# snap-research/GiGL

Measured on AMD Instinct MI355X. Metric: sampled+aggregated edges/s, higher is better.
Workload: dtype f32

## Files before the change

### gigl_amd/csrc/sample.hip

```cpp
#include "common.h"

#include <cstdlib>
#include <mutex>
#include <type_traits>

namespace {

constexpr uint64_t P1 = 0x9E3779B185EBCA87ULL;
constexpr uint64_t P2 = 0xC2B2AE3D27D4EB4FULL;
constexpr uint64_t P3 = 0x165667B19E3779F9ULL;
constexpr uint64_t P5 = 0x27D4EB2F165667C5ULL;
constexpr uint64_t SPARK_SEED = 42ULL;
constexpr uint64_t SIGN = 0x8000000000000000ULL;

__device__ __forceinline__ uint64_t xxh64_i32_ordered(uint32_t x) {
  uint64_t h = (SPARK_SEED + P5 + 4ULL) ^ ((uint64_t)x * P1);
  h = ((h << 23) | (h >> 41)) * P2 + P3;
  h ^= h >> 33;
  h *= P2;
  h ^= h >> 29;
  h *= P3;
  h ^= h >> 32;
  return h ^ SIGN;
}
// ... 225 lines not shown
    } else {
      const uint32_t ulo = dpp_shr1((uint32_t)key), uhi = dpp_shr1((uint32_t)(key >> 32));
      const uint32_t ui = dpp_shr1(idx), gtu = dpp_shr1(gt ? 1u : 0u);
      if (gtu) {
        key = ((uint64_t)uhi << 32) | ulo;
        idx = ui;
      } else if (gt) {
        key = ck;
        idx = ci;
      }
    }
  }
  __device__ __forceinline__ void merge(key_t ck, uint32_t ci, bool valid) {
    if constexpr (FAST) {
      if (__ballot(valid && ck == tk && tk != inf())) tie = true;
    }
    unsigned long long m = __ballot(valid && lt(ck, ci, tk, ti));
    while (m) {
      const int src = __ffsll((long long)m) - 1;
      m &= m - 1;
      const key_t sk = bcast(ck, src);
      const uint32_t si = readlane32(ci, src);
      if constexpr (FAST) {
        if (sk == tk) tie = true;
      }
      if (lt(sk, si, tk, ti)) {
        insert(sk, si);
        refresh_threshold();
      }
    }
  }
  __device__ __forceinline__ void scan_row(const uint32_t* flat, int64_t deg, uint32_t base) {
    const int64_t nchunks = (deg + 63) >> 6;
    const uint32_t* src = flat + base;
    auto key_at = [&](int64_t i) -> key_t {
      if constexpr (FAST) {
        if (flat) return i <= deg ? (key_t)(src[i] & dmask) : inf();
      }
      return mk(xxh64_i32_ordered((uint32_t)i + base));
    };
    int64_t c = 0;
    for (; c + 3 < nchunks; c += 4) {
      const int64_t ia = 1 + c * 64 + lane, ib = ia + 64, ic = ib + 64, id = ic + 64;
      const key_t ka = key_at(ia), kb = key_at(ib), kc = key_at(ic), kd = key_at(id);
      merge(ka, (uint32_t)ia, ia <= deg);
      merge(kb, (uint32_t)ib, ib <= deg);
      merge(kc, (uint32_t)ic, ic <= deg);
      merge(kd, (uint32_t)id, id <= deg);
    }
    for (; c < nchunks; ++c) {
      const int64_t i = 1 + c * 64 + lane;
      merge(key_at(i), (uint32_t)i, i <= deg);
    }
  }
  __device__ __forceinline__ bool scan_level(const RangeTable& tb, int l, uint32_t T, uint32_t n, uint32_t base) {
    const int gs = TBL_IDX_SHIFT + l;
    const uint32_t* off = tb.off[l];
    const uint2* ent = tb.lvl[l];
    const uint32_t start = off[(base + 1u) >> gs], end = off[((base + n) >> gs) + 1u];
    for (uint32_t e0 = start; e0 < end; e0 += 64u) {
      const uint32_t e = e0 + (uint32_t)lane;
      uint2 x = make_uint2(0u, 0xFFFFFFFFu);
      if (e < end) x = ent[e];
      const uint32_t i = x.x - base;
      const bool pass = e < end && (uint32_t)(i - 1u) < n && x.y < T;
      key_t ck;
      if constexpr (FAST) ck = x.y & dmask;
      else ck = xxh64_i32_ordered(x.x);
      merge(ck, i, pass);
    }
    return readlane32(idx, f - 1) != 0xFFFFFFFFu;
  }
  __device__ __forceinline__ bool finish(uint32_t count, uint32_t* lk, uint32_t* li) {
    if (count < (uint32_t)f || count > 64u) {
      wave_lds_sync();
      return false;
    }
    if (lane < 7) lk[count + (uint32_t)lane] = 0xFFFFFFFFu;
    wave_lds_sync();
    const bool valid = (uint32_t)lane < count;
    const uint32_t k = valid ? lk[lane] : 0xFFFFFFFFu;
    const uint32_t i = valid ? li[lane] : 0xFFFFFFFFu;
    uint32_t rank = 0;
    for (uint32_t j = 0; j < count; j += 8) {
      const uint4 q = *(const uint4*)(lk + j), r = *(const uint4*)(lk + j + 4);
      rank += (q.x < k ? 1u : 0u) + (q.y < k ? 1u : 0u) + (q.z < k ? 1u : 0u) + (q.w < k ? 1u : 0u);
      rank += (r.x < k ? 1u : 0u) + (r.y < k ? 1u : 0u) + (r.z < k ? 1u : 0u) + (r.w < k ? 1u : 0u);
    }
    wave_lds_sync();
    selmask = __ballot(valid && rank < (uint32_t)f);
    if (__popcll(selmask) != f) {
      tie = true;
      return true;
    }
    idx = i;
    ordered = true;
    return true;
  }
  __device__ __forceinline__ void offer(uint32_t k, uint32_t i, bool pass, uint32_t& count, uint32_t* lk, uint32_t* li) {
    const unsigned long long m = __ballot(pass);
    const uint32_t pos =
        count + __builtin_amdgcn_mbcnt_hi((uint32_t)(m >> 32), __builtin_amdgcn_mbcnt_lo((uint32_t)m, 0u));
    if (pass && pos < 64u) {
      lk[pos] = k;
      li[pos] = i;
    }
    count += (uint32_t)__popcll(m);
  }
  template <int SRC>
  __device__ __forceinline__ bool filter_positions(const uint32_t* flat, uint32_t n, uint32_t T, uint32_t base,
                                                   uint32_t* lk, uint32_t* li) {
    const bool all = T == 0xFFFFFFFFu;
    uint32_t count = 0;
    const uint32_t nchunks = (n + 63u) >> 6;
    const uint32_t* src = flat + base;
    for (uint32_t c = 0; c < nchunks; c += 4) {
      uint32_t kk[4];
#pragma unroll
      for (uint32_t t = 0; t < 4; ++t) {
        const uint32_t i = (c + t) * 64u + (uint32_t)lane + 1u;
        kk[t] = 0xFFFFFFFFu;
        if constexpr (SRC == SRC_FLAT) {
          if (c + t < nchunks) kk[t] = src[i];
        } else {
          kk[t] = (uint32_t)(xxh64_i32_ordered(i + base) >> 32);
        }
      }
#pragma unroll
      for (uint32_t t = 0; t < 4; ++t) {
        if (c + t >= nchunks) break;
        const uint32_t i = (c + t) * 64u + (uint32_t)lane + 1u;
        const uint32_t k = kk[t] & dmask;
        offer(k, i, i <= n && (all || k < T), count, lk, li);
      }
    }
    return finish(count, lk, li);
  }
  __device__ __forceinline__ bool filter_level(const uint2* ent, uint32_t cnt, uint32_t n, uint32_t T, uint32_t base,
                                               uint32_t* lk, uint32_t* li) {
    uint32_t count = 0;
    for (uint32_t e0 = 0; e0 < cnt; e0 += 128u) {
      const uint32_t ea = e0 + (uint32_t)lane, eb = ea + 64u;
      uint2 xa = make_uint2(0u, 0xFFFFFFFFu), xb = xa;
      if (ea < cnt) xa = ent[ea];
      if (eb < cnt) xb = ent[eb];
      const uint32_t ia = xa.x - base, ib = xb.x - base;
      offer(xa.y & dmask, ia, (uint32_t)(ia - 1u) < n && xa.y < T, count, lk, li);
      if (e0 + 64u < cnt) offer(xb.y & dmask, ib, (uint32_t)(ib - 1u) < n && xb.y < T, count, lk, li);
    }
    return finish(count, lk, li);
  }
  __device__ __forceinline__ void serial(const RangeTable& tb, uint32_t n, uint32_t base, uint32_t T, bool in_table) {
    reset_best();
    if (!in_table) {
      scan_row(nullptr, (int64_t)n, base);
      return;
    }
    const uint32_t T4 = T >= (1u << 30) ? 0xFFFFFFFFu : 4u * T;
    const int l4 = T4 == 0xFFFFFFFFu ? 0 : min((int)__builtin_clz(T4 - 1u), tb.levels);
    if (l4 > 0) {
      if (scan_level(tb, l4, T4, n, base)) return;
      reset_best();
    }
    if constexpr (FAST) {
      scan_row(tb.flat, (int64_t)n, base);
      if (readlane32(idx, f - 1) == 0xFFFFFFFFu) tie = true;
    } else {
      scan_row(nullptr, (int64_t)n, base);
    }
  }
};

enum { ROW_INVALID = 0, ROW_COPY = 1, ROW_FLAT = 2, ROW_LEVEL = 3, ROW_HASH = 4, ROW_SERIAL = 5, ROW_SERIAL_HASH = 6,
       ROW_SKIP = 7 };

struct __attribute__((aligned(32))) RowDesc {
  int64_t s;
  uint32_t n;
  uint32_t base;
  uint32_t T;
  uint32_t kind_cnt;
  const void* ptr;
};

__device__ __forceinline__ float filter_lambda(int f) { return (float)f + 4.f * __builtin_sqrtf((float)f) + 4.f; }

constexpr int WORK_LISTS = 64;
constexpr int WORK_CNT_STRIDE = 32;

struct WorkLists {
  uint32_t* items;
  int32_t* count;
  int64_t cap;
  int32_t iters;
  int32_t wgs;
};

__host__ __device__ static inline int64_t work_list_cap(int64_t n_parents) {
  return ((n_parents / 256 + 1 + WORK_LISTS - 1) / WORK_LISTS) * 256;
}
static inline int64_t expand_desc_bytes(int64_t n_parents) {
  return (n_parents + 1) * (int64_t)sizeof(RowDesc) + WORK_LISTS * work_list_cap(n_parents) * 4 +
         WORK_LISTS * WORK_CNT_STRIDE * 4 + 512;
}

__global__ void work_counts_zero_kernel(int32_t* count) { count[threadIdx.x * WORK_CNT_STRIDE] = 0; }

__global__ __launch_bounds__(256) void plan_rows_kernel(ExpandArgs a, RangeTable tb, RowDesc* __restrict__ desc,
                                                        int64_t* heavy_list, int32_t* heavy_count, WorkLists wl) {
  __shared__ int32_t s_wave[4];
  __shared__ int32_t s_base;
  const uint32_t p = blockIdx.x * 256u + threadIdx.x;
  const int lane = threadIdx.x & 63, w = threadIdx.x >> 6;
  bool real = false;
  if (p <= (uint32_t)a.n_parents) {
    RowDesc d{};
    if (p == (uint32_t)a.n_parents) {
      d.kind_cnt = ROW_SKIP;
      desc[p] = d;
    } else {
      uint32_t v, ksum;
      parent_of(a, p, v, ksum);
      uint32_t* out = a.out_nbr + (int64_t)p * a.f;
      if (v == GIGL_INVALID || (int64_t)v >= a.n_nodes) {
        for (int j = 0; j < a.f; ++j) out[j] = GIGL_INVALID;
        a.out_cnt[p] = 0;
      } else {
        int64_t deg;
        if (a.peer_world) {
          const uint32_t q = v / a.peer_world, rk = v - q * a.peer_world;
          const int64_t* rp = a.peer_rowptr[rk];
          const int64_t s0 = rp[q];
          deg = rp[q + 1] - s0;
          d.s = ((int64_t)rk << 48) | s0;
        } else {
          d.s = a.rowptr[v];
          deg = a.rowptr[v + 1] - d.s;
        }
        d.n = (uint32_t)deg;
        d.base = ksum + (uint32_t)a.hash_add;
        if (deg <= a.f && !a.multi) {
          const uint32_t* row = row_of_desc(a, d.s);
          for (int j = 0; j < a.f; ++j) out[j] = j < (int)deg ? row[j] : GIGL_INVALID;
          a.out_cnt[p] = (int32_t)deg;
        } else if (deg <= a.f) {
          d.kind_cnt = ROW_COPY;
          desc[p] = d;
          real = true;
        } else {
          const bool in_table = (uint64_t)d.base + (uint64_t)deg < tb.dom;
          const float lam = filter_lambda(a.f);
          d.T = d.n <= 64u ? 0xFFFFFFFFu
                           : (uint32_t)fminf(lam * 4294967296.f * __builtin_amdgcn_rcpf((float)d.n), 4294967040.f);
          uint32_t kind;
          if (!in_table) {
            if (deg > HEAVY_DEG) {
              kind = ROW_SKIP;
              if (heavy_list) heavy_list[atomicAdd(heavy_count, 1)] = (int64_t)p;
            } else {
              kind = lam <= 56.f ? ROW_HASH : ROW_SERIAL_HASH;
            }
          } else if (lam > 56.f) {
            kind = ROW_SERIAL;
          } else {
            const int l = min((int)__builtin_clz(d.T - 1u), tb.levels);
            if (l == 0 || d.n <= (uint32_t)a.flat_max) {
              kind = ROW_FLAT;
              d.ptr = tb.flat;
            } else {
              const int gs = TBL_IDX_SHIFT + l;
              const uint32_t* off = tb.off[l];
              const uint32_t start = off[(d.base + 1u) >> gs], end = off[((d.base + d.n) >> gs) + 1u];
              if (end - start > 256u) {
                kind = ROW_SERIAL;
              } else {
                kind = ROW_LEVEL | ((end - start) << 3);
                d.ptr = tb.lvl[l] + start;
              }
            }
          }
          d.kind_cnt = kind;
          desc[p] = d;
          real = (kind & 7u) != ROW_SKIP;
        }
      }
    }
  }
  const unsigned long long m = __ballot(real);
  if (lane == 0) s_wave[w] = (int32_t)__popcll(m);
  __syncthreads();
  const int list = (int)(blockIdx.x % WORK_LISTS);
  if (threadIdx.x == 0) {
    const int32_t tot = s_wave[0] + s_wave[1] + s_wave[2] + s_wave[3];
    s_base = tot ? atomicAdd(&wl.count[list * WORK_CNT_STRIDE], tot) : 0;
  }
  __syncthreads();
  if (real) {
    int32_t pos = s_base + (int32_t)__popcll(m & ((1ull << lane) - 1ull));
    for (int k = 0; k < w; ++k) pos += s_wave[k];
    wl.items[(int64_t)list * wl.cap + pos] = p;
  }
}

struct Cand {
  uint32_t k0, j0, k1, j1;
  bool ahead;
};

__device__ __forceinline__ Cand fetch_candidates(const RowDesc& d, int lane) {
  Cand c;
  c.k0 = c.k1 = 0xFFFFFFFFu;
  c.j0 = c.j1 = d.base;
  c.ahead = false;
  const uint32_t kind = d.kind_cnt & 7u, cnt = d.kind_cnt >> 3;
  if (kind == ROW_LEVEL && cnt <= 128u) {
    const uint2* ent = (const uint2*)d.ptr;
    if ((uint32_t)lane < cnt) {
      const uint2 x = ent[lane];
      c.j0 = x.x;
      c.k0 = x.y;
    }
    if ((uint32_t)lane + 64u < cnt) {
      const uint2 x = ent[lane + 64];
      c.j1 = x.x;
      c.k1 = x.y;
    }
    c.ahead = true;
  } else if (kind == ROW_FLAT && d.n <= 128u) {
    const uint32_t* src = (const uint32_t*)d.ptr + d.base;
    c.j0 = d.base + (uint32_t)lane + 1u;
    c.k0 = src[lane + 1];
    if (d.n > 64u) {
      c.j1 = c.j0 + 64u;
      c.k1 = src[lane + 65];
    }
    c.ahead = true;
  }
  return c;
}

__device__ __forceinline__ bool select_ahead(Sel<true>& sel, const RowDesc& d, const Cand& c, uint32_t* lk, uint32_t* li) {
  const uint32_t n = d.n, T = d.T, base = d.base;
  const bool all = T == 0xFFFFFFFFu;
  uint32_t count = 0;
  const uint32_t i0 = c.j0 - base, i1 = c.j1 - base;
  sel.offer(c.k0 & sel.dmask, i0, (uint32_t)(i0 - 1u) < n && (all || c.k0 < T), count, lk, li);
  if ((d.kind_cnt & 7u) == ROW_LEVEL ? (d.kind_cnt >> 3) > 64u : n > 64u)
    sel.offer(c.k1 & sel.dmask, i1, (uint32_t)(i1 - 1u) < n && (all || c.k1 < T), count, lk, li);
  return sel.finish(count, lk, li);
}

__global__ __launch_bounds__(256) __attribute__((amdgpu_waves_per_eu(8, 8))) void expand_rows_kernel(
    ExpandArgs a, RangeTable tb, const RowDesc* __restrict__ desc, WorkLists wl) {
  __shared__ __attribute__((aligned(16))) uint32_t s_lk[4][72], s_li[4][64];
  const int lane = threadIdx.x & 63;
  const int wave_in_block = __builtin_amdgcn_readfirstlane((int)(threadIdx.x >> 6));
  const int f = a.f;
  uint32_t* lk = s_lk[wave_in_block];
  uint32_t* li = s_li[wave_in_block];
  const uint32_t wgs_p = wl.iters > 0 ? (uint32_t)wl.wgs : gridDim.x;
  const uint32_t round = blockIdx.x / wgs_p;
  const uint32_t gw = (blockIdx.x % wgs_p) * 4u + (uint32_t)wave_in_block, n_waves = wgs_p * 4u;
  const uint32_t list = gw % WORK_LISTS, stride = n_waves / WORK_LISTS;
  const int32_t n_items = __builtin_amdgcn_readfirstlane(wl.count[list * WORK_CNT_STRIDE]);
  const uint32_t* items = wl.items + (int64_t)list * wl.cap;
  const uint32_t k_first = gw / WORK_LISTS + stride * round * (uint32_t)wl.iters;
  const uint32_t k_end = wl.iters > 0 ? k_first + stride * (uint32_t)wl.iters : 0xFFFFFFFFu;
  for (uint32_t k = k_first; (int32_t)(2u * k) < n_items && k < k_end; k += stride) {
    const uint32_t p0 = __builtin_amdgcn_readfirstlane(items[2u * k]);
    const uint32_t p1 = (int32_t)(2u * k + 1u) < n_items ? __builtin_amdgcn_readfirstlane(items[2u * k + 1u])
                                                         : (uint32_t)a.n_parents;
    const RowDesc d0 = desc[p0], d1 = desc[p1];
    const Cand c0 = fetch_candidates(d0, lane), c1 = fetch_candidates(d1, lane);
    Sel<true> s0, s1;
    s0.init(f, lane, a.proxy_drop);
    s1.init(f, lane, a.proxy_drop);
    const bool done0 = c0.ahead && !a.multi && select_ahead(s0, d0, c0, lk, li) && !s0.tie;
    uint32_t slot0 = 0, val0 = 0;
    bool sel0 = false;
    if (done0) {
      const unsigned long long m = s0.selmask;
      sel0 = (m >> lane) & 1ull;
      slot0 = __builtin_amdgcn_mbcnt_hi((uint32_t)(m >> 32), __builtin_amdgcn_mbcnt_lo((uint32_t)m, 0u));
      if (sel0) val0 = row_of_desc(a, d0.s)[s0.idx - 1];
    }
    const bool done1 = c1.ahead && !a.multi && select_ahead(s1, d1, c1, lk, li) && !s1.tie;
    uint32_t slot1 = 0, val1 = 0;
    bool sel1 = false;
    if (done1) {
      const unsigned long long m = s1.selmask;
      sel1 = (m >> lane) & 1ull;
      slot1 = __builtin_amdgcn_mbcnt_hi((uint32_t)(m >> 32), __builtin_amdgcn_mbcnt_lo((uint32_t)m, 0u));
      if (sel1) val1 = row_of_desc(a, d1.s)[s1.idx - 1];
    }
    if (done0) {
      if (sel0) a.out_nbr[(int64_t)p0 * f + slot0] = val0;
      if (lane == 0) a.out_cnt[p0] = f;
    }
    if (done1) {
      if (sel1) a.out_nbr[(int64_t)p1 * f + slot1] = val1;
      if (lane == 0) a.out_cnt[p1] = f;
    }
    if (done0 && done1) continue;
  #pragma nounroll
    for (int r = 0; r < 2; ++r) {
      if (r == 0 ? done0 : done1) continue;
      const RowDesc d = r == 0 ? d0 : d1;
      const uint32_t p = r == 0 ? p0 : p1;
      const uint32_t kind = d.kind_cnt & 7u;
      if (kind == ROW_SKIP) continue;
      uint32_t* out = a.out_nbr + (int64_t)p * f;
      if (kind == ROW_INVALID) {
        if (lane < f) out[lane] = GIGL_INVALID;
        if (lane == 0) a.out_cnt[p] = 0;
        continue;
      }
      const uint32_t* row = row_of_desc(a, d.s);
      const uint32_t n = d.n, base = d.base, T = d.T;
      if (kind == ROW_COPY) {
        if (a.multi) {
          const int nw = emit_sorted_distinct(row, (uint32_t)lane < n ? (uint32_t)lane + 1u : 0xFFFFFFFFu, f, lane, out);
          if (lane == 0) a.out_cnt[p] = nw;
          continue;
        }
        if (lane < f) out[lane] = (uint32_t)lane < n ? row[lane] : GIGL_INVALID;
        if (lane == 0) a.out_cnt[p] = (int32_t)n;
        continue;
      }
      const bool in_table = kind != ROW_HASH && kind != ROW_SERIAL_HASH;
      uint32_t sel_idx;
      {
        Sel<true> fast;
        fast.init(f, lane, a.proxy_drop);
        bool done = false;
        if (kind == ROW_LEVEL) done = fast.filter_level((const uint2*)d.ptr, d.kind_cnt >> 3, n, T, base, lk, li);
        else if (kind == ROW_FLAT) done = fast.template filter_positions<SRC_FLAT>((const uint32_t*)d.ptr, n, T, base, lk, li);
        else if (kind == ROW_HASH) done = fast.template filter_positions<SRC_HASH>(nullptr, n, T, base, lk, li);
        if (!done) fast.serial(tb, n, base, T, in_table);
        sel_idx = fast.idx;
        if (fast.tie) {
          Sel<false> exact;
          exact.init(f, lane);
          exact.serial(tb, n, base, T, in_table);
          sel_idx = exact.idx;
        } else if (fast.ordered) {
          const unsigned long long m = fast.selmask;
          const bool sel = (m >> lane) & 1ull;
          const uint32_t slot = __builtin_amdgcn_mbcnt_hi((uint32_t)(m >> 32), __builtin_amdgcn_mbcnt_lo((uint32_t)m, 0u));
          const uint32_t val = sel ? row[sel_idx - 1] : GIGL_INVALID;
          if (!a.multi) {
            if (sel) out[slot] = val;
            if (lane == 0) a.out_cnt[p] = f;
            continue;
          }
          if (sel) lk[slot] = val;
          wave_lds_sync();
          const bool keep = sel && (slot == 0 || lk[slot - 1] != val);
          wave_lds_sync();
          const unsigned long long km = __ballot(keep);
          if (lane < f) out[lane] = GIGL_INVALID;
          if (keep) out[__builtin_amdgcn_mbcnt_hi((uint32_t)(km >> 32), __builtin_amdgcn_mbcnt_lo((uint32_t)km, 0u))] = val;
          if (lane == 0) a.out_cnt[p] = (int32_t)__popcll(km);
          continue;
        }
      }
      if (a.multi) {
        const int nw = emit_sorted_distinct(row, sel_idx, f, lane, out);
        if (lane == 0) a.out_cnt[p] = nw;
        continue;
      }
      emit_sorted(row, sel_idx, f, lane, out);
      if (lane == 0) a.out_cnt[p] = f;
    }
    wave_lds_sync();
  }
}

__global__ __launch_bounds__(256) void table_flat_kernel(uint32_t* flat, uint64_t dom) {
  const uint64_t j = (uint64_t)blockIdx.x * 256 + threadIdx.x;
  if (j < dom) flat[j] = (uint32_t)(xxh64_i32_ordered((uint32_t)j) >> 32);
}

__device__ __forceinline__ int level_of(uint32_t proxy, int levels) { return min((int)__clz((int)proxy), levels); }

__global__ __launch_bounds__(256) void table_count_kernel(const uint32_t* flat, uint32_t* cnt, uint32_t n_tiles,
                                                          int levels) {
  __shared__ uint32_t s_cnt[TBL_MAX_LEVELS + 1][4];
  const int lane = threadIdx.x & 63, w = threadIdx.x >> 6;
  const uint32_t tile = blockIdx.x;
  const uint64_t j0 = ((uint64_t)tile << TBL_TILE_SHIFT) + (uint64_t)w * 256 + lane;
  int m[4];
#pragma unroll
  for (int r = 0; r < 4; ++r) m[r] = level_of(flat[j0 + r * 64], levels);
  for (int l = 1; l <= levels; ++l) {
    uint32_t c = 0;
#pragma unroll
    for (int r = 0; r < 4; ++r) c += (uint32_t)__popcll(__ballot(m[r] >= l));
    if (lane == 0) s_cnt[l][w] = c;
  }
  __syncthreads();
  const int l = threadIdx.x + 1;
  if (l <= levels) cnt[(uint64_t)(l - 1) * n_tiles + tile] = s_cnt[l][0] + s_cnt[l][1] + s_cnt[l][2] + s_cnt[l][3];
}

__global__ __launch_bounds__(1024) void table_scan_kernel(uint32_t* cnt, uint32_t n_tiles, uint32_t* total) {
  __shared__ uint32_t s_sum[1024];
  uint32_t* c = cnt + (uint64_t)blockIdx.x * n_tiles;
  const uint32_t span = (n_tiles + 1023u) / 1024u;
  const uint32_t lo = min(threadIdx.x * span, n_tiles), hi = min(lo + span, n_tiles);
  uint32_t s = 0;
  for (uint32_t t = lo; t < hi; ++t) s += c[t];
  s_sum[threadIdx.x] = s;
  __syncthreads();
  for (int d = 1; d < 1024; d <<= 1) {
    const uint32_t v = threadIdx.x >= (unsigned)d ? s_sum[threadIdx.x - d] : 0u;
    __syncthreads();
    s_sum[threadIdx.x] += v;
    __syncthreads();
  }
  uint32_t run = s_sum[threadIdx.x] - s;
  for (uint32_t t = lo; t < hi; ++t) {
    const uint32_t v = c[t];
    c[t] = run;
    run += v;
  }
  if (threadIdx.x == 1023) total[blockIdx.x + 1] = s_sum[1023];
}

struct TableBuild {
  const uint32_t* flat;
  const uint32_t* tile_off;
  const uint32_t* total;
  uint2* lvl[TBL_MAX_LEVELS + 1];
  uint32_t* off[TBL_MAX_LEVELS + 1];
  uint32_t n_tiles;
  int levels;
  uint64_t dom;
};

__global__ __launch_bounds__(256) void table_fill_kernel(TableBuild t) {
  __shared__ uint32_t s_cnt[TBL_MAX_LEVELS + 1][4];
  const int lane = threadIdx.x & 63, w = threadIdx.x >> 6;
  const uint32_t tile = blockIdx.x;
  const uint64_t jw = ((uint64_t)tile << TBL_TILE_SHIFT) + (uint64_t)w * 256;
  uint32_t px[4];
  int m[4];
#pragma unroll
  for (int r = 0; r < 4; ++r) {
    px[r] = t.flat[jw + r * 64 + lane];
    m[r] = level_of(px[r], t.levels);
  }
  for (int l = 1; l <= t.levels; ++l) {
    uint32_t c = 0;
#pragma unroll
    for (int r = 0; r < 4; ++r) c += (uint32_t)__popcll(__ballot(m[r] >= l));
    if (lane == 0) s_cnt[l][w] = c;
  }
  __syncthreads();
  for (int l = 1; l <= t.levels; ++l) {
    uint32_t run = t.tile_off[(uint64_t)(l - 1) * t.n_tiles + tile];
    for (int ww = 0; ww < w; ++ww) run += s_cnt[l][ww];
    const int gs = TBL_IDX_SHIFT + l;
    if (gs > TBL_TILE_SHIFT && s_cnt[l][w] == 0) continue;
#pragma unroll
    for (int r = 0; r < 4; ++r) {
      const unsigned long long mm = __ballot(m[r] >= l);
      const uint32_t before = run + __builtin_amdgcn_mbcnt_hi((uint32_t)(mm >> 32), __builtin_amdgcn_mbcnt_lo((uint32_t)mm, 0u));
      const uint64_t j = jw + r * 64 + lane;
      if (m[r] >= l) t.lvl[l][before] = make_uint2((uint32_t)j, px[r]);
      if (gs <= TBL_TILE_SHIFT && (j & ((1ull << gs) - 1)) == 0) t.off[l][j >> gs] = before;
      run += (uint32_t)__popcll(mm);
    }
  }
  if (threadIdx.x == 0) {
    const uint64_t j = (uint64_t)tile << TBL_TILE_SHIFT;
    for (int l = 1; l <= t.levels; ++l) {
      const int gs = TBL_IDX_SHIFT + l;
      if (gs > TBL_TILE_SHIFT && (j & ((1ull << gs) - 1)) == 0)
        t.off[l][j >> gs] = t.tile_off[(uint64_t)(l - 1) * t.n_tiles + tile];
      if (tile == t.n_tiles - 1) t.off[l][(t.dom + (1ull << gs) - 1) >> gs] = t.total[l];
    }
  }
}

__global__ __launch_bounds__(256) void expand_heavy_kernel(ExpandArgs a, const int64_t* heavy_list,
                                                           const int32_t* heavy_count) {
  __shared__ uint64_t s_key[4][64];
  __shared__ uint32_t s_idx[4][64];
  const int lane = threadIdx.x & 63;
  const int w = threadIdx.x >> 6;
  const int32_t n_heavy = *heavy_count;
  for (int32_t h = blockIdx.x; h < n_heavy; h += gridDim.x) {
    const int64_t p = heavy_list[h];
    uint32_t v, ksum;
    parent_of(a, p, v, ksum);
    const int f = a.f;
    const int64_t s = a.rowptr[v];
    const int64_t deg = a.rowptr[v + 1] - s;
    const uint32_t* row = a.col + s;
    const uint32_t base = ksum + (uint32_t)a.hash_add;
    uint32_t idx = 0xFFFFFFFFu;
    uint64_t key = ~0ULL;
    {
      uint64_t tk0 = ~0ULL;
      uint32_t ti0 = 0xFFFFFFFFu;
      scan_direct(key, idx, tk0, ti0, 1, deg, w, 4, base, f, lane);
    }
    s_key[w][lane] = key;
    s_idx[w][lane] = idx;
    __syncthreads();
    if (w == 0) {
      uint64_t tk = readlane64(key, f - 1);
      uint32_t ti = readlane32(idx, f - 1);
      for (int ow = 1; ow < 4; ++ow)
        merge_candidates(key, idx, s_key[ow][lane], s_idx[ow][lane], true, tk, ti, f, lane);
      if (a.multi) {
        const int nw = emit_sorted_distinct(row, idx, f, lane, a.out_nbr + p * f);
        if (lane == 0) a.out_cnt[p] = nw;
      } else {
        emit_sorted(row, idx, f, lane, a.out_nbr + p * f);
        if (lane == 0) a.out_cnt[p] = f;
      }
    }
    __syncthreads();
  }
}

constexpr int WIDE_CAP = 2048;

__device__ __forceinline__ void wide_bitonic(uint64_t* k, uint32_t* x, int cap, bool by_idx) {
  for (int size = 2; size <= cap; size <<= 1) {
    for (int stride = size >> 1; stride > 0; stride >>= 1) {
      __syncthreads();
      for (int t = threadIdx.x; t < cap / 2; t += blockDim.x) {
        const int lo = (t / stride) * (stride << 1) + (t % stride), hi = lo + stride;
        const bool up = (lo & size) == 0;
        const uint64_t ka = k[lo], kb = k[hi];
        const uint32_t xa = x[lo], xb = x[hi];
        const bool a_gt_b = by_idx ? (xa > xb) : less96(kb, xb, ka, xa);
        if (a_gt_b == up) {
          k[lo] = kb;
          k[hi] = ka;
          x[lo] = xb;
          x[hi] = xa;
        }
      }
    }
  }
  __syncthreads();
}

__global__ __launch_bounds__(256) void expand_wide_kernel(ExpandArgs a) {
  __shared__ uint64_t s_key[WIDE_CAP];
  __shared__ uint32_t s_idx[WIDE_CAP];
  __shared__ int32_t s_count;
  __shared__ int32_t s_scan[256];
  const int tid = threadIdx.x;
  const int f = a.f;
  for (int64_t p = blockIdx.x; p < a.n_parents; p += gridDim.x) {
    uint32_t v, ksum;
    parent_of(a, (uint32_t)p, v, ksum);
    uint32_t* out = a.out_nbr + p * f;
    __syncthreads();
    if (v == GIGL_INVALID || (int64_t)v >= a.n_nodes) {
      for (int j = tid; j < f; j += 256) out[j] = GIGL_INVALID;
      if (tid == 0) a.out_cnt[p] = 0;
      continue;
    }
    const int64_t s = a.rowptr[v];
    const int64_t deg = a.rowptr[v + 1] - s;
    const uint32_t* row = a.col + s;
    const uint32_t base = ksum + (uint32_t)a.hash_add;
    int n_sel;
    if (deg <= f) {
      for (int j = tid; j < f; j += 256) s_idx[j] = j < deg ? (uint32_t)(j + 1) : 0xFFFFFFFFu;
      n_sel = (int)deg;
      __syncthreads();
    } else {
      const double lam = (double)f + 6.0 * sqrt((double)f) + 16.0;
      double frac = lam / (double)deg;
      for (;;) {
        const uint64_t T = frac >= 1.0 ? ~0ULL : (uint64_t)(frac * 18446744073709551616.0);
        if (tid == 0) s_count = 0;
        __syncthreads();
        for (int64_t i = 1 + tid; i <= deg; i += 256) {
          const uint64_t key = xxh64_i32_ordered((uint32_t)i + base);
          if (key < T || T == ~0ULL) {
            const int slot = atomicAdd(&s_count, 1);
            if (slot < WIDE_CAP) {
              s_key[slot] = key;
              s_idx[slot] = (uint32_t)i;
            }
          }
        }
        __syncthreads();
        const int count = s_count;
        __syncthreads();
        if (count > WIDE_CAP) {
          frac *= 0.5;
          continue;
        }
        if (count < f) {
          frac *= 2.0;
          continue;
        }
        for (int j = count + tid; j < WIDE_CAP; j += 256) {
          s_key[j] = ~0ULL;
          s_idx[j] = 0xFFFFFFFFu;
        }
        int cap = 64;
        while (cap < count) cap <<= 1;
        wide_bitonic(s_key, s_idx, cap, false);
        int cap2 = 64;
        while (cap2 < f) cap2 <<= 1;
        for (int j = f + tid; j < cap2; j += 256) {
          s_key[j] = ~0ULL;
          s_idx[j] = 0xFFFFFFFFu;
        }
        wide_bitonic(s_key, s_idx, cap2, true);
        break;
      }
      n_sel = f;
    }
    int kept = 0;
    if (!a.multi) {
      for (int j = tid; j < f; j += 256) out[j] = j < n_sel ? row[s_idx[j] - 1] : GIGL_INVALID;
      kept = n_sel;
    } else {
      int run = 0;
      const int per = (f + 255) / 256;
      const int j0 = tid * per;
      for (int j = j0; j < j0 + per && j < n_sel; ++j) {
        const uint32_t val = row[s_idx[j] - 1];
        run += (j == 0 || row[s_idx[j - 1] - 1] != val) ? 1 : 0;
      }
      s_scan[tid] = run;
      __syncthreads();
      int off = 0;
      for (int t = 0; t < tid; ++t) off += s_scan[t];
      int total = 0;
      for (int t = 0; t < 256; ++t) total += s_scan[t];
      for (int j = j0; j < j0 + per && j < n_sel; ++j) {
        const uint32_t val = row[s_idx[j] - 1];
        if (j == 0 || row[s_idx[j - 1] - 1] != val) out[off++] = val;
      }
      for (int j = total + tid; j < f; j += 256) out[j] = GIGL_INVALID;
      kept = total;
    }
    if (tid == 0) a.out_cnt[p] = kept;
  }
}

struct TableOwner {
  RangeTable t{};
  void* mem = nullptr;
  void* mem2 = nullptr;
  int device = 0;
  int refs = 0;
};

std::mutex g_table_mu;
TableOwner* g_device_table[64] = {nullptr};

void table_unref(TableOwner* own) {
  if (!own || --own->refs > 0) return;
  if (g_device_table[own->device] == own) g_device_table[own->device] = nullptr;
  if (own->mem) hipFree(own->mem);
  if (own->mem2) hipFree(own->mem2);
  delete own;
}

uint64_t table_cap_j() {
  if (const char* e = getenv("GIGL_TABLE_MAX_J")) {
    const unsigned long long v = strtoull(e, nullptr, 10);
    if (v >= 64) return (uint64_t)v;
  }
  uint64_t cap = 1ull << 30;
// ... 511 lines not shown
```

Before: 11.12 billion.

## Software-pipeline work-item and row-descriptor loads in expand_rows_kernel

The expand loop now prefetches work items two iterations ahead and row descriptors one iteration ahead. Each descriptor is loaded as one dword per lane across 16 lanes and unpacked with readlane, replacing scalar struct loads. Candidate fetching is made branchless with clamped addresses and global address-space casts, and the slow general path moves into a separate inlined function that reloads its descriptor. The aim is to hide the latency of the dependent item, descriptor and candidate loads, at the cost of extra VGPR pressure, explicit waitcnt and asm barriers, and the layout assumptions pinned by static_asserts.

```diff
diff --git a/gigl_amd/csrc/sample.hip b/gigl_amd/csrc/sample.hip
--- a/gigl_amd/csrc/sample.hip
+++ b/gigl_amd/csrc/sample.hip
@@ -551,57 +551,157 @@
   }
 }
 
+template <class T>
+__device__ __forceinline__ const T* as_global(const void* p) {
+  return (const T*)(const __attribute__((address_space(1))) T*)(uintptr_t)p;
+}
+
+__device__ __forceinline__ uint32_t desc_n(uint32_t dv, int o) { return readlane32(dv, o + 2); }
+__device__ __forceinline__ uint32_t desc_base(uint32_t dv, int o) { return readlane32(dv, o + 3); }
+__device__ __forceinline__ uint32_t desc_T(uint32_t dv, int o) { return readlane32(dv, o + 4); }
+__device__ __forceinline__ uint32_t desc_kind_cnt(uint32_t dv, int o) { return readlane32(dv, o + 5); }
+__device__ __forceinline__ int64_t desc_s(uint32_t dv, int o) {
+  return (int64_t)(((uint64_t)readlane32(dv, o + 1) << 32) | readlane32(dv, o));
+}
+__device__ __forceinline__ const void* desc_ptr(uint32_t dv, int o) {
+  return (const void*)(uintptr_t)(((uint64_t)readlane32(dv, o + 7) << 32) | readlane32(dv, o + 6));
+}
+__device__ __forceinline__ RowDesc desc_unpack(uint32_t dv, int o) {
+  RowDesc d;
+  d.s = desc_s(dv, o);
+  d.n = desc_n(dv, o);
+  d.base = desc_base(dv, o);
+  d.T = desc_T(dv, o);
+  d.kind_cnt = desc_kind_cnt(dv, o);
+  d.ptr = desc_ptr(dv, o);
+  return d;
+}
+static_assert(sizeof(RowDesc) == 32 && offsetof(RowDesc, n) == 8 && offsetof(RowDesc, base) == 12 &&
+                  offsetof(RowDesc, T) == 16 && offsetof(RowDesc, kind_cnt) == 20 && offsetof(RowDesc, ptr) == 24,
+              "desc_* read RowDesc by dword");
+
 struct Cand {
   uint32_t k0, j0, k1, j1;
-  bool ahead;
+  int mode;
 };
+enum { CAND_NONE = 0, CAND_LEVEL = 1, CAND_FLAT = 2 };
 
 __device__ __forceinline__ Cand fetch_candidates(const RowDesc& d, int lane) {
   Cand c;
-  c.k0 = c.k1 = 0xFFFFFFFFu;
-  c.j0 = c.j1 = d.base;
-  c.ahead = false;
   const uint32_t kind = d.kind_cnt & 7u, cnt = d.kind_cnt >> 3;
-  if (kind == ROW_LEVEL && cnt <= 128u) {
-    const uint2* ent = (const uint2*)d.ptr;
-    if ((uint32_t)lane < cnt) {
-      const uint2 x = ent[lane];
-      c.j0 = x.x;
-      c.k0 = x.y;
-    }
-    if ((uint32_t)lane + 64u < cnt) {
-      const uint2 x = ent[lane + 64];
-      c.j1 = x.x;
-      c.k1 = x.y;
-    }
-    c.ahead = true;
-  } else if (kind == ROW_FLAT && d.n <= 128u) {
-    const uint32_t* src = (const uint32_t*)d.ptr + d.base;
-    c.j0 = d.base + (uint32_t)lane + 1u;
-    c.k0 = src[lane + 1];
-    if (d.n > 64u) {
-      c.j1 = c.j0 + 64u;
-      c.k1 = src[lane + 65];
-    }
-    c.ahead = true;
+  c.mode = kind == ROW_LEVEL && cnt - 1u < 128u ? CAND_LEVEL : kind == ROW_FLAT && d.n <= 128u ? CAND_FLAT : CAND_NONE;
+  c.k0 = c.j0 = c.k1 = c.j1 = 0u;
+  if (c.mode != CAND_NONE) {
+    const bool level = c.mode == CAND_LEVEL;
+    const char* pj = (const char*)as_global<uint32_t>(d.ptr) + (level ? 0u : 4u * (uint64_t)d.base);
+    const char* pk = pj + 4;
+    const uint32_t o0 = level ? 8u * min((uint32_t)lane, cnt - 1u) : 4u * (uint32_t)lane;
+    const uint32_t o1 = level ? 8u * min((uint32_t)lane + 64u, cnt - 1u) : 4u * (uint32_t)lane + 256u;
+    c.k0 = *(const uint32_t*)(pk + o0);
+    if (level) c.j0 = *(const uint32_t*)(pj + o0);
+    if (level ? cnt > 64u : d.n > 64u) {
+      c.k1 = *(const uint32_t*)(pk + o1);
+      if (level) c.j1 = *(const uint32_t*)(pj + o1);
+    }
   }
   return c;
 }
 
-__device__ __forceinline__ bool select_ahead(Sel<true>& sel, const RowDesc& d, const Cand& c, uint32_t* lk, uint32_t* li) {
-  const uint32_t n = d.n, T = d.T, base = d.base;
-  const bool all = T == 0xFFFFFFFFu;
+__device__ __forceinline__ bool select_ahead(Sel<true>& sel, const RowDesc& d, const Cand& c, uint32_t* lk, uint32_t* li,
+                                             int lane) {
+  const uint32_t n = d.n, T = d.T, base = d.base, cnt = d.kind_cnt >> 3;
+  const bool all = T == 0xFFFFFFFFu, level = c.mode == CAND_LEVEL;
   uint32_t count = 0;
-  const uint32_t i0 = c.j0 - base, i1 = c.j1 - base;
-  sel.offer(c.k0 & sel.dmask, i0, (uint32_t)(i0 - 1u) < n && (all || c.k0 < T), count, lk, li);
-  if ((d.kind_cnt & 7u) == ROW_LEVEL ? (d.kind_cnt >> 3) > 64u : n > 64u)
-    sel.offer(c.k1 & sel.dmask, i1, (uint32_t)(i1 - 1u) < n && (all || c.k1 < T), count, lk, li);
+  const uint32_t i0 = level ? c.j0 - base : (uint32_t)lane + 1u, i1 = level ? c.j1 - base : (uint32_t)lane + 65u;
+  const bool in0 = !level || (uint32_t)lane < cnt, in1 = !level || (uint32_t)lane + 64u < cnt;
+  sel.offer(c.k0 & sel.dmask, i0, in0 && (uint32_t)(i0 - 1u) < n && (all || c.k0 < T), count, lk, li);
+  if (level ? cnt > 64u : n > 64u)
+    sel.offer(c.k1 & sel.dmask, i1, in1 && (uint32_t)(i1 - 1u) < n && (all || c.k1 < T), count, lk, li);
   return sel.finish(count, lk, li);
+}
+
+__device__ __forceinline__ void expand_general(const ExpandArgs& a, const RangeTable& tb, const RowDesc* __restrict__ desc,
+                                               uint32_t p0, uint32_t p1, bool done0, bool done1, uint32_t* lk,
+                                               uint32_t* li, int lane) {
+  const int f = a.f;
+#pragma nounroll
+  for (int r = 0; r < 2; ++r) {
+    if (r == 0 ? done0 : done1) continue;
+    const uint32_t p = r == 0 ? p0 : p1;
+    const RowDesc d = desc[p];
+    const uint32_t kind = d.kind_cnt & 7u;
+    if (kind == ROW_SKIP) continue;
+    uint32_t* out = a.out_nbr + (int64_t)p * f;
+    if (kind == ROW_INVALID) {
+      if (lane < f) out[lane] = GIGL_INVALID;
+      if (lane == 0) a.out_cnt[p] = 0;
+      continue;
+    }
+    const uint32_t* row = as_global<uint32_t>(row_of_desc(a, d.s));
+    const uint32_t n = d.n, base = d.base, T = d.T;
+    if (kind == ROW_COPY) {
+      if (a.multi) {
+        const int nw = emit_sorted_distinct(row, (uint32_t)lane < n ? (uint32_t)lane + 1u : 0xFFFFFFFFu, f, lane, out);
+        if (lane == 0) a.out_cnt[p] = nw;
+        continue;
+      }
+      if (lane < f) out[lane] = (uint32_t)lane < n ? row[lane] : GIGL_INVALID;
+      if (lane == 0) a.out_cnt[p] = (int32_t)n;
+      continue;
+    }
+    const bool in_table = kind != ROW_HASH && kind != ROW_SERIAL_HASH;
+    uint32_t sel_idx;
+    {
+      Sel<true> fast;
+      fast.init(f, lane, a.proxy_drop);
+      bool done = false;
+      if (kind == ROW_LEVEL) done = fast.filter_level(as_global<uint2>(d.ptr), d.kind_cnt >> 3, n, T, base, lk, li);
+      else if (kind == ROW_FLAT) done = fast.template filter_positions<SRC_FLAT>(as_global<uint32_t>(d.ptr), n, T, base, lk, li);
+      else if (kind == ROW_HASH) done = fast.template filter_positions<SRC_HASH>(nullptr, n, T, base, lk, li);
+      if (!done) fast.serial(tb, n, base, T, in_table);
+      sel_idx = fast.idx;
+      if (fast.tie) {
+        Sel<false> exact;
+        exact.init(f, lane);
+        exact.serial(tb, n, base, T, in_table);
+        sel_idx = exact.idx;
+      } else if (fast.ordered) {
+        const unsigned long long m = fast.selmask;
+        const bool sel = (m >> lane) & 1ull;
+        const uint32_t slot = __builtin_amdgcn_mbcnt_hi((uint32_t)(m >> 32), __builtin_amdgcn_mbcnt_lo((uint32_t)m, 0u));
+        const uint32_t val = sel ? row[sel_idx - 1] : GIGL_INVALID;
+        if (!a.multi) {
+          if (sel) out[slot] = val;
+          if (lane == 0) a.out_cnt[p] = f;
+          continue;
+        }
+        if (sel) lk[slot] = val;
+        wave_lds_sync();
+        const bool keep = sel && (slot == 0 || lk[slot - 1] != val);
+        wave_lds_sync();
+        const unsigned long long km = __ballot(keep);
+        if (lane < f) out[lane] = GIGL_INVALID;
+        if (keep) out[__builtin_amdgcn_mbcnt_hi((uint32_t)(km >> 32), __builtin_amdgcn_mbcnt_lo((uint32_t)km, 0u))] = val;
+        if (lane == 0) a.out_cnt[p] = (int32_t)__popcll(km);
+        continue;
+      }
+    }
+    if (a.multi) {
+      const int nw = emit_sorted_distinct(row, sel_idx, f, lane, out);
+      if (lane == 0) a.out_cnt[p] = nw;
+      continue;
+    }
+    emit_sorted(row, sel_idx, f, lane, out);
+    if (lane == 0) a.out_cnt[p] = f;
+  }
+  wave_lds_sync();
+  __builtin_amdgcn_s_waitcnt(0x0F70);
 }
 
 __global__ __launch_bounds__(256) __attribute__((amdgpu_waves_per_eu(8, 8))) void expand_rows_kernel(
     ExpandArgs a, RangeTable tb, const RowDesc* __restrict__ desc, WorkLists wl) {
   __shared__ __attribute__((aligned(16))) uint32_t s_lk[4][72], s_li[4][64];
+  typedef uint32_t u32x2 __attribute__((ext_vector_type(2)));
   const int lane = threadIdx.x & 63;
   const int wave_in_block = __builtin_amdgcn_readfirstlane((int)(threadIdx.x >> 6));
   const int f = a.f;
@@ -611,37 +711,65 @@
   const uint32_t round = blockIdx.x / wgs_p;
   const uint32_t gw = (blockIdx.x % wgs_p) * 4u + (uint32_t)wave_in_block, n_waves = wgs_p * 4u;
   const uint32_t list = gw % WORK_LISTS, stride = n_waves / WORK_LISTS;
-  const int32_t n_items = __builtin_amdgcn_readfirstlane(wl.count[list * WORK_CNT_STRIDE]);
-  const uint32_t* items = wl.items + (int64_t)list * wl.cap;
+  const u32x2* items = reinterpret_cast<const u32x2*>(wl.items + (int64_t)list * wl.cap);
+  const uint32_t last_pair = (uint32_t)(wl.cap >> 1) - 1u;
+  const uint32_t skip = (uint32_t)a.n_parents;
   const uint32_t k_first = gw / WORK_LISTS + stride * round * (uint32_t)wl.iters;
   const uint32_t k_end = wl.iters > 0 ? k_first + stride * (uint32_t)wl.iters : 0xFFFFFFFFu;
-  for (uint32_t k = k_first; (int32_t)(2u * k) < n_items && k < k_end; k += stride) {
-    const uint32_t p0 = __builtin_amdgcn_readfirstlane(items[2u * k]);
-    const uint32_t p1 = (int32_t)(2u * k + 1u) < n_items ? __builtin_amdgcn_readfirstlane(items[2u * k + 1u])
-                                                         : (uint32_t)a.n_parents;
-    const RowDesc d0 = desc[p0], d1 = desc[p1];
+  auto vec = [](uint32_t x) -> uint32_t {
+    asm("" : "+v"(x));
+    return x;
+  };
+  auto load_items = [&](uint32_t k) -> u32x2 { return items[vec(min(k, last_pair))]; };
+  int32_t n_items = 0;
+  auto parents_of = [&](uint32_t k, u32x2 it, uint32_t& p0, uint32_t& p1) {
+    const uint32_t x = __builtin_amdgcn_readfirstlane(it.x), y = __builtin_amdgcn_readfirstlane(it.y);
+    p0 = (int32_t)(2u * k) < n_items ? x : skip;
+    p1 = (int32_t)(2u * k + 1u) < n_items ? y : skip;
+  };
+  const uint32_t* desc_w = reinterpret_cast<const uint32_t*>(desc);
+  auto load_desc = [&](uint32_t p0, uint32_t p1) -> uint32_t {
+    return desc_w[(uint64_t)((lane & 8) ? p1 : p0) * 8u + (uint32_t)(lane & 7)];
+  };
+  uint32_t k = k_first;
+  const u32x2 it_a = load_items(k), it_b = load_items(k + stride);
+  n_items = __builtin_amdgcn_readfirstlane(wl.count[list * WORK_CNT_STRIDE]);
+  if (!((int32_t)(2u * k) < n_items)) return;
+  uint32_t p0, p1, p0n, p1n;
+  parents_of(k, it_a, p0, p1);
+  parents_of(k + stride, it_b, p0n, p1n);
+  uint32_t dv = load_desc(p0, p1);
+  __builtin_amdgcn_s_waitcnt(0x0F70);
+  for (;;) {
+    const uint32_t kn = k + stride;
+    const u32x2 it_nn = load_items(kn + stride);
+    const uint32_t dvn = load_desc(p0n, p1n);
+    const RowDesc d0 = desc_unpack(dv, 0), d1 = desc_unpack(dv, 8);
     const Cand c0 = fetch_candidates(d0, lane), c1 = fetch_candidates(d1, lane);
     Sel<true> s0, s1;
     s0.init(f, lane, a.proxy_drop);
     s1.init(f, lane, a.proxy_drop);
-    const bool done0 = c0.ahead && !a.multi && select_ahead(s0, d0, c0, lk, li) && !s0.tie;
+    const bool done0 = c0.mode != CAND_NONE && !a.multi && select_ahead(s0, d0, c0, lk, li, lane) && !s0.tie;
+    uint32_t p0nn, p1nn;
+    parents_of(kn + stride, it_nn, p0nn, p1nn);
     uint32_t slot0 = 0, val0 = 0;
     bool sel0 = false;
     if (done0) {
       const unsigned long long m = s0.selmask;
       sel0 = (m >> lane) & 1ull;
       slot0 = __builtin_amdgcn_mbcnt_hi((uint32_t)(m >> 32), __builtin_amdgcn_mbcnt_lo((uint32_t)m, 0u));
-      if (sel0) val0 = row_of_desc(a, d0.s)[s0.idx - 1];
-    }
-    const bool done1 = c1.ahead && !a.multi && select_ahead(s1, d1, c1, lk, li) && !s1.tie;
+      if (sel0) val0 = as_global<uint32_t>(row_of_desc(a, d0.s))[s0.idx - 1];
+    }
+    const bool done1 = c1.mode != CAND_NONE && !a.multi && select_ahead(s1, d1, c1, lk, li, lane) && !s1.tie;
     uint32_t slot1 = 0, val1 = 0;
     bool sel1 = false;
     if (done1) {
       const unsigned long long m = s1.selmask;
       sel1 = (m >> lane) & 1ull;
       slot1 = __builtin_amdgcn_mbcnt_hi((uint32_t)(m >> 32), __builtin_amdgcn_mbcnt_lo((uint32_t)m, 0u));
-      if (sel1) val1 = row_of_desc(a, d1.s)[s1.idx - 1];
-    }
+      if (sel1) val1 = as_global<uint32_t>(row_of_desc(a, d1.s))[s1.idx - 1];
+    }
+    asm volatile("" ::"v"(val0), "v"(val1));
     if (done0) {
       if (sel0) a.out_nbr[(int64_t)p0 * f + slot0] = val0;
       if (lane == 0) a.out_cnt[p0] = f;
@@ -650,78 +778,14 @@
       if (sel1) a.out_nbr[(int64_t)p1 * f + slot1] = val1;
       if (lane == 0) a.out_cnt[p1] = f;
     }
-    if (done0 && done1) continue;
-  #pragma nounroll
-    for (int r = 0; r < 2; ++r) {
-      if (r == 0 ? done0 : done1) continue;
-      const RowDesc d = r == 0 ? d0 : d1;
-      const uint32_t p = r == 0 ? p0 : p1;
-      const uint32_t kind = d.kind_cnt & 7u;
-      if (kind == ROW_SKIP) continue;
-      uint32_t* out = a.out_nbr + (int64_t)p * f;
-      if (kind == ROW_INVALID) {
-        if (lane < f) out[lane] = GIGL_INVALID;
-        if (lane == 0) a.out_cnt[p] = 0;
-        continue;
-      }
-      const uint32_t* row = row_of_desc(a, d.s);
-      const uint32_t n = d.n, base = d.base, T = d.T;
-      if (kind == ROW_COPY) {
-        if (a.multi) {
-          const int nw = emit_sorted_distinct(row, (uint32_t)lane < n ? (uint32_t)lane + 1u : 0xFFFFFFFFu, f, lane, out);
-          if (lane == 0) a.out_cnt[p] = nw;
-          continue;
-        }
-        if (lane < f) out[lane] = (uint32_t)lane < n ? row[lane] : GIGL_INVALID;
-        if (lane == 0) a.out_cnt[p] = (int32_t)n;
-        continue;
-      }
-      const bool in_table = kind != ROW_HASH && kind != ROW_SERIAL_HASH;
-      uint32_t sel_idx;
-      {
-        Sel<true> fast;
-        fast.init(f, lane, a.proxy_drop);
-        bool done = false;
-        if (kind == ROW_LEVEL) done = fast.filter_level((const uint2*)d.ptr, d.kind_cnt >> 3, n, T, base, lk, li);
-        else if (kind == ROW_FLAT) done = fast.template filter_positions<SRC_FLAT>((const uint32_t*)d.ptr, n, T, base, lk, li);
-        else if (kind == ROW_HASH) done = fast.template filter_positions<SRC_HASH>(nullptr, n, T, base, lk, li);
-        if (!done) fast.serial(tb, n, base, T, in_table);
-        sel_idx = fast.idx;
-        if (fast.tie) {
-          Sel<false> exact;
-          exact.init(f, lane);
-          exact.serial(tb, n, base, T, in_table);
-          sel_idx = exact.idx;
-        } else if (fast.ordered) {
-          const unsigned long long m = fast.selmask;
-          const bool sel = (m >> lane) & 1ull;
-          const uint32_t slot = __builtin_amdgcn_mbcnt_hi((uint32_t)(m >> 32), __builtin_amdgcn_mbcnt_lo((uint32_t)m, 0u));
-          const uint32_t val = sel ? row[sel_idx - 1] : GIGL_INVALID;
-          if (!a.multi) {
-            if (sel) out[slot] = val;
-            if (lane == 0) a.out_cnt[p] = f;
-            continue;
-          }
-          if (sel) lk[slot] = val;
-          wave_lds_sync();
-          const bool keep = sel && (slot == 0 || lk[slot - 1] != val);
-          wave_lds_sync();
-          const unsigned long long km = __ballot(keep);
-          if (lane < f) out[lane] = GIGL_INVALID;
-          if (keep) out[__builtin_amdgcn_mbcnt_hi((uint32_t)(km >> 32), __builtin_amdgcn_mbcnt_lo((uint32_t)km, 0u))] = val;
-          if (lane == 0) a.out_cnt[p] = (int32_t)__popcll(km);
-          continue;
-        }
-      }
-      if (a.multi) {
-        const int nw = emit_sorted_distinct(row, sel_idx, f, lane, out);
-        if (lane == 0) a.out_cnt[p] = nw;
-        continue;
-      }
-      emit_sorted(row, sel_idx, f, lane, out);
-      if (lane == 0) a.out_cnt[p] = f;
-    }
-    wave_lds_sync();
+    if (!(done0 && done1)) expand_general(a, tb, desc, p0, p1, done0, done1, lk, li, lane);
+    if (!((int32_t)(2u * kn) < n_items && kn < k_end)) break;
+    k = kn;
+    p0 = p0n;
+    p1 = p1n;
+    p0n = p0nn;
+    p1n = p1nn;
+    dv = dvn;
   }
 }
 
```

Result: faster. 11.54 billion, median of 6 (+3.8%).
